# SYNCC-IN/hyperscanning-signal-analysis

Measured on AMD Instinct MI355X. Metric: MVAR+ffDTF windows/sec, 2x32-ch dyad p=8, 256 freqs, higher is better.
Workload: dtype f64; 1 GPU; C2: 1 dyad(s)/GPU, 2x32 ch @500 Hz, 10 min, 2 s windows 50% overlap (599 windows per dyad), MVAR p=8, 256 freqs 0.5-128 Hz; dyads_per_gpu=1, k1=hop blocks summed once, shared by the overlapping windows (hop 500), k2=block Levinson-Whittle recursion, one workgroup per window, one launch, normalisation=inside K3 (rows of window w by workgroups of window w+lag), parallelism=dyad-sharded x1, gather=none

## Files before the change

hyperscanning_signal_analysis_amd/csrc/tf_inv.hip:

```cpp
#include "hmv_common.h"
#include "hmv_kernels.h"

namespace hmv {

#ifndef HMV_K3_WGS
#define HMV_K3_WGS 4
#endif

#ifndef HMV_ROW_LOADS_SC1
#define HMV_ROW_LOADS_SC1 0
#endif

#define HMV_LDS_FENCE()                                     \
  do {                                                      \
    __builtin_amdgcn_fence(__ATOMIC_RELEASE, "wavefront");  \
    __builtin_amdgcn_wave_barrier();                        \
    __builtin_amdgcn_fence(__ATOMIC_ACQUIRE, "wavefront");  \
  } while (0)

#ifdef HMV_STAMP
#define HMV_T(idx)                                                                     \
  do {                                                                                 \
    __builtin_amdgcn_sched_barrier(0);                                                 \
    unsigned long long t_;                                                             \
    asm volatile("s_memtime %0\n\ts_waitcnt lgkmcnt(0)" : "=s"(t_)::"memory");          \
    __builtin_amdgcn_sched_barrier(0);                                                 \
    tsum[idx] += t_ - tlast;                                                           \
    tlast = t_;                                                                        \
  } while (0)
#else
#define HMV_T(idx) do { } while (0)
#endif

template <int NT>
struct TfLds {
  static constexpr int MP = 16 * NT;
  static constexpr int NRING = 3;
  static constexpr int PBUF = MP * 5;
  static constexpr int NBUF = MP * 4;
  static constexpr int SROW = 8;
  static constexpr int SWAPB = NT * 32;
  static constexpr int RSUM = NT * MP / 2;
  static constexpr int TOTAL = PBUF + NRING * NBUF + SROW + SWAPB + RSUM;
};

typedef double f64x2 __attribute__((ext_vector_type(2)));
__device__ __forceinline__ void store_sc1_b128(double* p, f64x2 v) {
  asm volatile("global_store_dwordx4 %0, %1, off sc1\n\ts_nop 1" ::"v"(p), "v"(v) : "memory");
}
__device__ __forceinline__ void store_sc1_b64(double* p, double v) {
  asm volatile("global_store_dwordx2 %0, %1, off sc1" ::"v"(p), "v"(v) : "memory");
}

template <int NT>
struct NormLds {
  static constexpr int MP = 16 * NT;
  static constexpr int FC = 16, JC = (MP % 32 == 0) ? 32 : 16, TS = JC + 1;
  static constexpr int DOUBLES = NT * FC * TS + 5 * MP;
};

template <int NT>
__device__ __forceinline__ void window_denominators(const TfArgs& a, int item, double* lds, const int tid) {
  constexpr int MP = 16 * NT;
  using N = NormLds<NT>;
  double* dpart = lds + NT * N::FC * N::TS;
  const int F = a.F, t = tid;
  const int ty = t / MP, tx = t - ty * MP;
  const double* rs = a.rowsum + (size_t)item * F * MP + tx;
  const int fq = (F + 3) >> 2;
  const int f1 = min(F, (ty + 1) * fq);
  double acc = 0.0;
  int f = ty * fq;
  for (; f + 16 <= f1; f += 16) {
    double v[16];
#pragma unroll
    for (int k = 0; k < 16; ++k) v[k] = rs[(size_t)(f + k) * MP];
#pragma unroll
    for (int k = 0; k < 16; ++k) acc += v[k];
  }
  for (; f < f1; ++f) acc += rs[(size_t)f * MP];
  dpart[ty * MP + tx] = acc;
  __syncthreads();
  if (t < MP) {
    const double d = ((dpart[t] + dpart[MP + t]) + dpart[2 * MP + t]) + dpart[3 * MP + t];
    store_sc1_b64(a.den + (size_t)item * MP + t, d);
  }
}

template <int NT>
__device__ __forceinline__ void normalise_row(const TfArgs& a, int item, int i, double* lds, const int tid) {
  constexpr int MP = 16 * NT;
  using N = NormLds<NT>;
  constexpr int FC = N::FC, JC = N::JC, TS = N::TS;
  constexpr int J2 = JC / 2, FR = 64 / J2, NL = FC / FR, NQ = JC / 8, NJC = MP / JC, D = 4;
  const int F = a.F, m = a.m;
  const int l = tid & 63, wv = uni(tid >> 6);
  double* tile = lds + wv * (FC * TS);
  const double r = 1.0 / __hip_atomic_load(a.den + (size_t)item * MP + i, __ATOMIC_RELAXED, __HIP_MEMORY_SCOPE_AGENT);
  const int total = (F / FC) * NJC;
  const int fr = l / J2, j2 = l - fr * J2;
  const int f2 = l & 7, jr = l >> 3;
#if !HMV_ROW_LOADS_SC1
  const double* Pw = a.P + ((size_t)item * MP + i) * F * MP + (size_t)fr * MP + 2 * j2;
#endif
  double* ow = a.ff + ((size_t)item * m + i) * m * F + (size_t)jr * F + 2 * f2;
#if HMV_ROW_LOADS_SC1
  const double* slab = a.P + ((size_t)item * MP + i) * F * MP;
  const __amdgpu_buffer_rsrc_t rs = __builtin_amdgcn_make_buffer_rsrc(const_cast<double*>(slab), 0, F * MP * 8, 0x00020000);
  const int off0 = (fr * MP + 2 * j2) * 8;
#endif
  auto issue = [&](f64x2 (&v)[NL], int u) __attribute__((always_inline)) {
    if (u < total) {
      const int jc = u % NJC, f0 = (u / NJC) * FC;
#if HMV_ROW_LOADS_SC1
      const int off = off0 + (f0 * MP + jc * JC) * 8;
#pragma unroll
      for (int k = 0; k < NL; ++k)
        v[k] = __builtin_bit_cast(f64x2, __builtin_amdgcn_raw_buffer_load_b128(rs, off + k * FR * MP * 8, 0, 16 ));
#else
      const double* src = Pw + (size_t)f0 * MP + jc * JC;
#pragma unroll
      for (int k = 0; k < NL; ++k)
        v[k] = __builtin_nontemporal_load(reinterpret_cast<const f64x2*>(src + (size_t)(k * FR) * MP));
#endif
    }
  };
  auto drain = [&](const f64x2 (&v)[NL], int u) __attribute__((always_inline)) {
    if (u < total) {
      const int jc = u % NJC, f0 = (u / NJC) * FC, j0 = jc * JC;
#pragma unroll
      for (int k = 0; k < NL; ++k) {
        double* w = tile + (fr + k * FR) * TS + 2 * j2;
        w[0] = v[k].x;
        w[1] = v[k].y;
      }
      HMV_LDS_FENCE();
      double* dst = ow + (size_t)j0 * F + f0;
#pragma unroll
      for (int q = 0; q < NQ; ++q) {
        const double x0 = tile[(2 * f2) * TS + jr + 8 * q], x1 = tile[(2 * f2 + 1) * TS + jr + 8 * q];
        f64x2 o;
        o.x = x0 * r;
        o.y = x1 * r;
        if (j0 + jr + 8 * q < m) __builtin_nontemporal_store(o, reinterpret_cast<f64x2*>(dst + (size_t)(8 * q) * F));
      }
      HMV_LDS_FENCE();
    }
  };
  f64x2 buf[D][NL];
  static_for<D>([&](auto dc) __attribute__((always_inline)) { issue(buf[decltype(dc)::value], wv + NT * decltype(dc)::value); });
  for (int u = wv; u < total; u += NT * D) {
    static_for<D>([&](auto dc) __attribute__((always_inline)) {
      constexpr int d = decltype(dc)::value;
      drain(buf[d], u + NT * d);
      issue(buf[d], u + NT * (d + D));
    });
  }
}

template <int NT>
__device__ __forceinline__ void band_row(const TfArgs& a, int item, int i, double* lds, const int lds_doubles, const int tid) {
  constexpr int MP = 16 * NT, NBP = 5, D = 4;
  const int F = a.F, m = a.m, nb = a.nb;
  const int l = tid & 63, wv = uni(tid >> 6);
  const int c = l & 15, jl = 8 * wv + 2 * (l >> 4);
  const double r = 1.0 / __hip_atomic_load(a.den + (size_t)item * MP + i, __ATOMIC_RELAXED, __HIP_MEMORY_SCOPE_AGENT);
  const int fit = lds_doubles / F;
  const int nbp = fit < NBP ? fit : NBP;
  const int nk = F >> 5;
  for (int b0 = 0; b0 < nb; b0 += nbp) {
    __syncthreads();
    for (int e = tid; e < nbp * F; e += 64 * NT) {
      const int b = e / F, f = e - b * F, bb = b0 + b;
      lds[e] = (bb < nb && f >= a.band_lo[bb] && f < a.band_hi[bb]) ? 1.0 : 0.0;
    }
    __syncthreads();
    const double* wl = lds + 2 * c;
// ... 68 lines not shown
    else normalise_row<NT>(a, item, i, lds, (int)threadIdx.x);
    __syncthreads();
  }
}

template <int NT, bool GEN, bool BANDS = true>
__device__ __forceinline__ void tf_outputs(const TfArgs& a, const int item, const int f, const long long gw, const int w,
                                           const int wv, double (&re)[NT][4], double (&im)[NT][4], double2* smem,
                                           double* rsum, const int* s_orig, int* s_flag, const double* s_det
#ifdef HMV_STAMP
                                           , unsigned long long (&tsum)[8], unsigned long long& tlast
#endif
) {
  constexpr int MP = 16 * NT, NG = NT;
  using L = TfLds<NT>;
  constexpr int NR = L::NRING;
  int& s_info = *s_flag;
  int lo;
  asm volatile("v_mbcnt_lo_u32_b32 %0, -1, 0\n\tv_mbcnt_hi_u32_b32 %0, -1, %0" : "=v"(lo));
  const int rowo = 4 * ((lo >> 2) & 3) + (lo >> 4), jo = lo & 3;
  const int tid = 64 * wv + lo;
  int oc[4];
#pragma unroll
  for (int Jl = 0; Jl < 4; ++Jl) oc[Jl] = s_orig[4 * (Jl * NT + w) + jo];
  if (w == 0 && lo == 0) {
    a.info[gw] = s_info;
    if constexpr (GEN) {
      if (a.detph) {
        a.detph[2 * gw] = s_det[0];
        a.detph[2 * gw + 1] = s_det[1];
      }
    }
  }

  if (a.H) {
    double2* Ho = reinterpret_cast<double2*>(a.H) + (size_t)gw * MP * MP + (size_t)rowo * MP;
#pragma unroll
    for (int Ig = 0; Ig < NG; ++Ig)
#pragma unroll
      for (int Jl = 0; Jl < 4; ++Jl) Ho[(size_t)(16 * Ig) * MP + oc[Jl]] = make_double2(re[Ig][Jl], im[Ig][Jl]);
  }
  if (a.P) {
    double* rs = rsum + w * MP + rowo;
    const bool publish = !GEN && (a.ff != nullptr || a.bands != nullptr) && item < a.fuse_items;
    if (!publish) {
      double* Po = a.P + (size_t)gw * MP * MP + (size_t)rowo * MP;
#pragma unroll
      for (int Ig = 0; Ig < NG; ++Ig) {
        double acc = 0.0;
#pragma unroll
        for (int Jl = 0; Jl < 4; ++Jl) {
          const double v = re[Ig][Jl] * re[Ig][Jl] + im[Ig][Jl] * im[Ig][Jl];
          Po[(size_t)(16 * Ig) * MP + oc[Jl]] = v;
          acc += v;
        }
        acc += dpp_f64<0xB1>(acc);
        acc += dpp_f64<0x4E>(acc);
        if (jo == 0) rs[16 * Ig] = acc;
      }
      __syncthreads();
      if (w == 0 && lo < MP) {
        double t = 0.0;
#pragma unroll
        for (int ww = 0; ww < NT; ++ww) t += rsum[ww * MP + lo];
        a.rowsum[(size_t)gw * MP + lo] = t;
      }
    } else {
      constexpr int G = (NT == 3) ? 1 : (NT == 4 ? 2 : NT), TS = MP + 2, C2 = MP / 2, CNT = 16 * G * C2;
      static_assert(16 * G * TS <= 2 * (L::PBUF + NR * L::NBUF + L::SROW + L::SWAPB), "publish tile overlaps the row sums");
      double* tile = reinterpret_cast<double*>(smem);
      double* Pg = a.P + (size_t)item * MP * a.F * MP + (size_t)f * MP;
      static_for<NG / G>([&](auto pc) __attribute__((always_inline)) {
        constexpr int pass = decltype(pc)::value;
        if (pass > 0) __syncthreads();
        static_for<G>([&](auto gc) __attribute__((always_inline)) {
          constexpr int g = decltype(gc)::value, Ig = pass * G + g;
          double acc = 0.0;
#pragma unroll
          for (int Jl = 0; Jl < 4; ++Jl) {
            const double v = re[Ig][Jl] * re[Ig][Jl] + im[Ig][Jl] * im[Ig][Jl];
            tile[(16 * g + rowo) * TS + oc[Jl]] = v;
            acc += v;
          }
          acc += dpp_f64<0xB1>(acc);
          acc += dpp_f64<0x4E>(acc);
          if (jo == 0) rs[16 * Ig] = acc;
        });
        __syncthreads();
#pragma unroll
        for (int idx = tid; idx < CNT; idx += 64 * NT) {
          const int row = idx / C2, c2 = idx - row * C2;
          const f64x2 v = *reinterpret_cast<const f64x2*>(tile + row * TS + 2 * c2);
          store_sc1_b128(Pg + (size_t)(16 * G * pass + row) * a.F * MP + 2 * c2, v);
        }
      });
      if (w == 0 && lo < MP) {
        double t = 0.0;
#pragma unroll
        for (int ww = 0; ww < NT; ++ww) t += rsum[ww * MP + lo];
        store_sc1_b64(a.rowsum + (size_t)gw * MP + lo, t);
      }
    }
  }
  HMV_T(4);

  if constexpr (!GEN) {
    if (a.ff != nullptr || a.bands != nullptr) {
      static_assert(NormLds<NT>::DOUBLES <= 2 * L::TOTAL, "normaliser tiles do not fit the inversion's LDS block");
      double* nlds = reinterpret_cast<double*>(smem);
      if (item < a.fuse_items) {
        asm volatile("s_waitcnt vmcnt(0)" ::: "memory");
        __syncthreads();
        if (tid == 0) {
          const int old = __hip_atomic_fetch_add(a.wcount + item, 1, __ATOMIC_RELAXED, __HIP_MEMORY_SCOPE_AGENT);
          const int last = (old == a.F - 1) ? 1 : 0;
          if (last) {
            __builtin_amdgcn_fence(__ATOMIC_ACQUIRE, "agent");
            asm volatile("s_waitcnt vmcnt(0)" ::: "memory");
          }
          s_info = last;
        }
        __syncthreads();
        HMV_T(5);
        if (s_info != 0) {
          window_denominators<NT>(a, item, nlds, tid);
          asm volatile("s_waitcnt vmcnt(0)" ::: "memory");
          __syncthreads();
          if (tid == 0) __hip_atomic_store(a.ready + item, 1, __ATOMIC_RELAXED, __HIP_MEMORY_SCOPE_AGENT);
        }
      }
      const int wl = item - a.lag;
      if (wl >= 0 && wl < a.fuse_items - a.lag && f < a.m) {
        __syncthreads();
        if (tid == 0) {
          const int rdy = __hip_atomic_load(a.ready + wl, __ATOMIC_RELAXED, __HIP_MEMORY_SCOPE_AGENT);
          if (!rdy) {
            for (int i = f; i < a.m; i += a.F) {
              const int pos = __hip_atomic_fetch_add(a.missed, 1, __ATOMIC_RELAXED, __HIP_MEMORY_SCOPE_AGENT);
              a.missed[1 + pos] = wl * MP + i;
            }
          }
          s_info = rdy;
        }
        __syncthreads();
        HMV_T(6);
        if (s_info != 0) {
          if (BANDS && a.bands) {
            if constexpr (BANDS)
              for (int i = f; i < a.m; i += a.F) band_row<NT>(a, wl, i, nlds, 2 * L::TOTAL, tid);
          } else {
            for (int i = f; i < a.m; i += a.F) normalise_row<NT>(a, wl, i, nlds, tid);
          }
        }
      }
    }
  }
#ifdef HMV_STAMP
  HMV_T(7);
  if (a.stamps && lo == 0) {
    for (int k = 0; k < 8; ++k) a.stamps[(gw * NT + wv) * 8 + k] = tsum[k];
  }
#endif
}

template <int NT, bool GEN>
__global__ void __launch_bounds__(64 * NT, (NT == 4) ? HMV_K3_WGS : 2) tf_inv_kernel(TfArgs a) {
  constexpr int MP = 16 * NT, NG = NT, NSTEP = MP / 4;
  using L = TfLds<NT>;
  constexpr int NR = L::NRING;
  __shared__ double2 smem[L::TOTAL];
  __shared__ int s_orig[MP];
  __shared__ __attribute__((aligned(16))) int s_swp[NR][4];
  __shared__ int s_info;
  __shared__ double s_det[2];

  const int l = lane_id();
  const int wv = uni(threadIdx.x >> 6);
  const unsigned bid = blockIdx.x + (unsigned)a.item0 * (unsigned)a.F;
  const int w = (wv + (int)((bid * 2654435761u) >> 20)) % NT;
  const int item = uni((int)(bid / (unsigned)a.F));
  const int f = uni((int)(bid - (unsigned)item * (unsigned)a.F));
  const long long gw = (long long)item * a.F + f;
  const int p = a.p;
  const int i = l >> 4, b = (l >> 2) & 3, j = l & 3;
  const int rowl = 4 * b + i;
  const int colw = 4 * w + j;

  double2* Pbuf = smem;
  double2* Nbuf = Pbuf + L::PBUF;
  double2* Srow = Nbuf + NR * L::NBUF;
  double2* swapb = Srow + L::SROW + wv * 32;
// ... 611 lines not shown
```

hyperscanning_signal_analysis_amd/_lib.py:

```python
from __future__ import annotations

import ctypes
import os
from ctypes import POINTER, c_char_p, c_double, c_int, c_int32, c_int64, c_void_p

_HERE = os.path.dirname(os.path.abspath(__file__))
LIB_PATH = os.path.join(_HERE, "libhypermvar.so")

SIGNATURES = {
    "hmv_version": (c_int, []),
    "hmv_last_error": (c_char_p, []),
    "hmv_pad": (c_int, [c_int]),
    "hmv_set_tuning": (c_int, [c_int, c_int64]),
    "hmv_get_tuning": (c_int64, [c_int]),
    "hmv_yw_workspace_doubles": (c_int64, [c_int, c_int]),
    "hmv_lagcov_f64": (c_int, [c_void_p, c_int64, c_int64, c_void_p, c_void_p, c_int64, c_int, c_int, c_int,
                               c_void_p, c_void_p]),
    "hmv_lagcov_regular_workspace_doubles": (c_int64, [c_int64, c_int, c_int, c_int64, c_int]),
    "hmv_lagcov_regular_f64": (c_int, [c_void_p, c_int64, c_int64, c_int64, c_int64, c_int64, c_int, c_int, c_int,
                                       c_void_p, c_void_p, c_void_p]),
    "hmv_yw_solve_f64": (c_int, [c_void_p, c_int64, c_int, c_int, c_void_p, c_void_p, c_void_p, c_void_p,
                                 c_void_p, c_int64, c_void_p]),
    "hmv_yw_routes_i32": (c_int, [c_void_p, c_int64, c_int, c_int, c_void_p, c_void_p]),
    "hmv_twiddles_f64": (c_int, [c_void_p, c_int, c_double, c_int, c_void_p, c_void_p]),
# ... 107 lines not shown
    "hmv_surrogate_phase_c128": (c_int, [c_void_p, c_int64, c_void_p, c_int, c_int, c_int, c_void_p, c_void_p]),
    "hmv_null_accumulate_f64": (c_int, [c_void_p, c_void_p, c_void_p, c_void_p, c_int64, c_int, c_int, c_int] + [c_void_p] * 12),
    "hmv_residuals_workspace_bytes": (c_int64, [c_int64, c_int, c_int]),
    "hmv_residuals_f64": (c_int, [c_void_p, c_int64, c_int64, c_void_p, c_void_p, c_int64, c_int, c_int, c_int, c_void_p,
                                  c_void_p, c_int64, c_void_p, c_int64, c_void_p]),
    "hmv_whiteness_f64": (c_int, [c_void_p, c_int64, c_int, c_int, c_int, c_double] + [c_void_p] * 6),
    "hmv_model_validation_workspace_bytes": (c_int64, [c_int64, c_int, c_int, c_int, c_int]),
    "hmv_model_validation_f64": (c_int, [c_void_p, c_int64, c_int64, c_void_p, c_void_p, c_int64, c_int, c_int, c_int,
                                         c_void_p, c_int, c_double] + [c_void_p] * 7 + [c_int64, c_void_p, c_int64, c_int64,
                                                                                       c_void_p]),
    "hmv_decimate_out_len": (c_int64, [c_int64, c_int]),
    "hmv_decimate_tile": (c_int, [c_int, c_int]),
    "hmv_decimate_fir_f64": (c_int, [c_void_p, c_int64, c_int64, c_int64, c_int64, c_int, c_int, c_void_p, c_int, c_void_p,
                                     c_int64, c_int64, c_void_p]),
    "hmv_phase_sync_c128": (c_int, [c_void_p, c_int64, c_int64, c_int64, c_int64, c_int, c_void_p, c_void_p, c_int64, c_int, c_int,
                                    c_void_p, c_void_p, c_void_p, c_void_p, c_void_p]),
}

FLAG_UNFUSED_NORM = 1
FLAG_YW_TILED = 2
FLAG_YW_ONE_LAUNCH = 4
FLAG_DIRECT_LAGCOV = 8
FLAG_YW_PIVOTED = 16
MEASURE_FFDTF = 0
MEASURE_DDTF = 1
MEASURE_GPDC = 2
CRITERIA = {"AIC": 0, "HQ": 1, "SC": 2}
TUNE_NORM_LAG = 1
TUNE_LAG_GROUP = 2
TUNE_K3_FORM = 3
TUNE_YW_FORM = 4
TUNE_K3_LDS_PAD = 5
TUNE_K3_SPLIT = 6
MAX_DECIMATE = 32
MAX_DECIMATE_TAPS = 641
PHASE_UNIT = 0
PHASE_RAW = 1


_lib = None


class HypermvarLibraryError(ImportError):
    pass


def load():
    global _lib
    if _lib is not None:
        return _lib
    global LIB_PATH
    LIB_PATH = os.environ.get("HYPERMVAR_LIB", LIB_PATH)
    if not os.path.exists(LIB_PATH):
        raise HypermvarLibraryError(
            f"{LIB_PATH} not found: build the HIP library first "
            f"(python -c 'import __graft_entry__ as g; g.build()' or make -C {_HERE}/csrc). "
            "There is no CPU fallback for the MVAR/ffDTF path.")
    lib = ctypes.CDLL(LIB_PATH)
    for name, (res, args) in SIGNATURES.items():
        try:
            fn = getattr(lib, name)
        except AttributeError as e:
            raise HypermvarLibraryError(f"{LIB_PATH} does not export {name}") from e
        fn.restype = res
        fn.argtypes = args
    _lib = lib
# ... 11 lines not shown
```

hyperscanning_signal_analysis_amd/csrc/capi.hip:

```cpp
#include "../../include/hypermvar.h"
#include "hmv_kernels.h"

#include <atomic>
#include <cmath>
#include <cstdio>
#include <cstdlib>
#include <cstring>

namespace {
thread_local char g_err[256] = "";

int fail(int code, const char* msg) {
  snprintf(g_err, sizeof(g_err), "%s", msg);
  return code;
}
int refuse(const char* who, int code, const char* msg) {
  snprintf(g_err, sizeof(g_err), "%s: %s", who, msg);
  return code;
}
int pad_of(int m) { return (m < 1 || m > HMV_MAX_CHANNELS) ? -1 : ((m + 15) / 16) * 16; }
inline hipStream_t S(void* s) { return reinterpret_cast<hipStream_t>(s); }
inline size_t align256(size_t b) { return (b + 255) & ~size_t(255); }

constexpr int N_TUNE = 7;
// ... 619 lines not shown
  return w;
}
struct BgcWs {
  size_t off_B, off_C, off_D, off_cst, off_Ra, off_Rb, off_arr, off_Vra, off_Vrb, off_ir, off_full, total;
};
BgcWs bgc_layout(size_t front, int64_t chunk, int m, int p, int F, int split, bool bands, bool time, bool spectral = true) {
  BgcWs w;
  size_t o = front;
  const hmv::BgcPads pd = hmv::bgc_pads(m, split);
  const size_t mp = (size_t)pad_of(m), mpa = (size_t)pd.mpa, mpb = (size_t)pd.mpb, nsp = (size_t)pd.nsp, pp = (size_t)p + 1;
  w.off_B = o;      if (spectral) o += align256(sizeof(double) * chunk * pp * mp * mp);
  w.off_C = o;      if (spectral) o += align256(sizeof(double) * chunk * 2 * pp * nsp * nsp);
  w.off_D = o;      if (spectral) o += align256(sizeof(double) * chunk * 2 * pp * nsp * nsp);
  w.off_cst = o;    if (spectral) o += align256(sizeof(double) * chunk * 2);
  w.off_Ra = o;     if (time) o += align256(sizeof(double) * chunk * pp * mpa * mpa);
  w.off_Rb = o;     if (time) o += align256(sizeof(double) * chunk * pp * mpb * mpb);
  w.off_arr = o;    if (time) o += align256(sizeof(double) * chunk * nsp * nsp * p);
  w.off_Vra = o;    if (time) o += align256(sizeof(double) * chunk * mpa * mpa);
  w.off_Vrb = o;    if (time) o += align256(sizeof(double) * chunk * mpb * mpb);
  w.off_ir = o;     if (time) o += align256(sizeof(int32_t) * chunk * 2);
  w.off_full = o;   if (bands) o += align256(sizeof(double) * chunk * 2 * F);
  w.total = o;
  return w;
}
int64_t sliding_bytes(int64_t chunk, int m, int p, int F, int n_bands = 0, bool spectra = false, int measure = MEAS_FFDTF,
                      int64_t q_tiles = -1) {
  const int mp = pad_of(m);
  if (mp < 0 || chunk < 1 || p < 1 || p > HMV_MAX_ORDER || F < 1 || n_bands < 0 || measure < MEAS_FFDTF ||
      measure > MEAS_GPDC)
    return -1;
  return (int64_t)sliding_layout(chunk, mp, p, F, n_bands > 0, spectra, measure, q_tiles).total;
}
struct ForkJoin {
  hipEvent_t fork = nullptr, join = nullptr;
};
ForkJoin* fork_join_events() {
  constexpr int MAXDEV = 64;
  thread_local ForkJoin tl[MAXDEV];
  int dev = 0;
  if (hipGetDevice(&dev) != hipSuccess || dev < 0 || dev >= MAXDEV) return nullptr;
  ForkJoin& e = tl[dev];
  if (!e.fork) {
    if (hipEventCreateWithFlags(&e.fork, hipEventDisableTiming) != hipSuccess) return nullptr;
    if (hipEventCreateWithFlags(&e.join, hipEventDisableTiming) != hipSuccess) return nullptr;
  }
  return &e;
}
int64_t k3_split_point(int64_t c, int mp, int64_t lag) {
  const int64_t t = hmv::tuning(HMV_TUNE_K3_SPLIT);
  int64_t c0 = t;
  if (t < 0) return 0;
  if (t == 0) {
    constexpr int MAXDEV = 64;
    struct Shape { int cus = 0, occ[4] = {0, 0, 0, 0}; };
    thread_local Shape tl[MAXDEV];
    int dev = 0;
    if (hipGetDevice(&dev) != hipSuccess || dev < 0 || dev >= MAXDEV || mp < 16 || mp > 64) return 0;
    Shape& d = tl[dev];
    int& occ = d.occ[mp / 16 - 1];
    if (d.cus == 0 && hipDeviceGetAttribute(&d.cus, hipDeviceAttributeMultiprocessorCount, dev) != hipSuccess) d.cus = -1;
    if (occ == 0 && (occ = hmv::yw_lwr_occupancy(mp)) == 0) occ = -1;
    if (d.cus < 1 || occ < 1) {
      (void)hipGetLastError();
      return 0;
    }
    const int64_t k = c / d.cus, r = c % d.cus;
    if (k < 1 || k >= occ || r == 0) return 0;
    c0 = c - r;
  }
  return (c0 >= lag && c0 < c) ? c0 : 0;
}
}

int64_t hmv_sliding_workspace_bytes(int64_t chunk, int m, int p, int F) { return sliding_bytes(chunk, m, p, F); }

namespace {
struct MixDesc {
  const double* Rt;
  const double* W;
  const double* scale;
  int64_t n_trials, n_win, n_mix;
};
struct BgcDesc {
  int split;
  double* time;
  int32_t* info_red;
  int32_t* info_gc;
  int want = 3;
  double* red_out = nullptr;
  const double* red_base = nullptr;
  const int32_t* info_red_base = nullptr;
};
struct Items {
  const double* x;
  int64_t rec_stride, ld;
  const int64_t* item_rec;
  const int64_t* item_start;
  int64_t n_items;
  int m, n, p;
};
struct Grid { int64_t hop, first, nwin, T; };
struct Spectral { const double* freqs; int F; double fs; };
struct Output {
// ... 39 lines not shown
  Run run;
  OrderSel sel = {};
  const EnsDesc* ens = nullptr;
  const PairDesc* pairs = nullptr;
  const MixDesc* mix = nullptr;
  const BgcDesc* bgc = nullptr;
};

int measure_request(const char* who, int measure, int n_bands, const double* S_out, FitOut& fit, int crit = 0) {
  if (measure < HMV_MEASURE_FFDTF || measure > HMV_MEASURE_GPDC)
    return refuse(who, -4, "measure must be HMV_MEASURE_FFDTF, _DDTF or _GPDC");
  if (crit < 0 || crit > 2) return refuse(who, -5, "criterion must be 0 (AIC), 1 (HQ) or 2 (SC)");
  if (n_bands < 0) return refuse(who, -4, "n_bands must be >= 0");
  if (S_out && (measure != HMV_MEASURE_FFDTF || n_bands != 0))
    return refuse(who, -4, "spectra come with the full ffDTF only");
  if (measure == HMV_MEASURE_GPDC) { fit.info_tf = nullptr; fit.pivot_tau = 1.0; }
  return 0;
}
int need_output(const char* who, const void* out, int64_t n_items) {
  return (!out && n_items != 0) ? refuse(who, -4, "null pointer / empty grid") : 0;
}
int need_output_after_sizes(const char* who, const Items& it, const void* out) {
  const bool sizes_ok = pad_of(it.m) >= 0 && it.p >= 1 && it.p <= HMV_MAX_ORDER && it.n > it.p;
  return sizes_ok ? need_output(who, out, it.n_items) : 0;
}
int64_t measure_bytes(int measure, int64_t chunk, int m, int p, int F, int n_bands, int64_t q_tiles) {
  const bool spectra = (n_bands == -1 && measure == HMV_MEASURE_FFDTF);
  return sliding_bytes(chunk, m, p, F, spectra ? 0 : n_bands, spectra, measure, q_tiles);
}

struct TwoStreams {
  hipStream_t st0 = nullptr, st1 = nullptr;
  ForkJoin* ev = nullptr;
  int fork() const {
    const int hrc = (int)hipEventRecord(ev->fork, st0);
    return hrc ? hrc : (int)hipStreamWaitEvent(st1, ev->fork, 0);
  }
  int record_join() const {
    const int hrc = (int)hipEventRecord(ev->join, st1);
    if (hrc) (void)hipStreamSynchronize(st1);
    return hrc;
  }
  int wait_join(hipEvent_t join) const {
    const int hrc = (int)hipStreamWaitEvent(st0, join, 0);
    if (hrc) (void)hipStreamSynchronize(st1);
    return hrc;
  }
  int join() const {
    const int hrc = record_join();
    return hrc ? hrc : wait_join(ev->join);
  }
  void finish(hmv::TfSplit& sp) const {
    if (sp.join && !sp.joined) (void)wait_join(sp.join);
    sp.joined = true;
  }
};

struct SlidingPlan {
  bool empty = false;
  int mp = 0;
  size_t t = 0, ws_item = 0;
  bool automatic = false, bands = false, k3_bands = false, bgc_spec = false, bgc_time = false;
  bool regular = false, ens_shared = false;
  bool ldl = false, from_tiles = false;
  bool half_split = false, k3_split = false;
  TwoStreams fj;
  SlidingWs w{};
  BgcWs gw{};
  char* base = nullptr;
  double *R = nullptr, *Qb = nullptr, *ws = nullptr, *ar = nullptr, *V = nullptr, *den = nullptr, *tw = nullptr;
// ... 96 lines not shown

int sliding_k1(const SlidingArgs& a, const SlidingPlan& pl, const Chunk& ch) {
  const Items& it = a.it;
  const int64_t i0 = ch.i0, c = ch.c;
  hipStream_t st = pl.fj.st0;
  const K1In in{it.x, it.rec_stride, it.ld, it.item_rec, it.item_start, it.m, it.n, it.p};
  if (a.ens) {
    const hmv::LagcovEnsArgs ea = ens_args(in, *a.ens, i0, c, pl.R, pl.ens_shared ? pl.Qb : nullptr, a.grid.hop, a.grid.nwin);
    return a.ens->split ? hmv::launch_lagcov_ensemble_split(ea, pl.mp, st)
                        : hmv::launch_lagcov_ensemble(ea, pl.mp, pl.ens_shared, st);
  }
  if (a.pairs) return hmv::launch_lagcov_pairs(pairs_args(in, *a.pairs, i0, c, pl.R), pl.mp, st);
  if (a.mix) {
    hmv::LagcovMixArgs ma{};
    ma.Rt = a.mix->Rt; ma.W = a.mix->W; ma.scale = a.mix->scale; ma.n_trials = a.mix->n_trials; ma.n_win = a.mix->n_win;
    ma.it0 = i0; ma.n_items = c; ma.m = it.m; ma.m_pad = pl.mp; ma.p = it.p; ma.R = pl.R;
    return hmv::launch_lagcov_mix(ma, st);
  }
  if (!pl.regular)
    return hmv_lagcov_f64(it.x, it.rec_stride, it.ld, it.item_rec + i0, it.item_start + i0, c, it.m, it.n, it.p, pl.R, st);
  const Grid& g = a.grid;
  const size_t stack = (size_t)(it.p + 1) * pl.t;
  int rc = 0;
  for (int64_t k = i0; k < i0 + c && rc == 0;) {
    const int64_t rec = k / g.nwin, w0 = k - rec * g.nwin;
    const int64_t run = ((g.nwin - w0) < (i0 + c - k)) ? (g.nwin - w0) : (i0 + c - k);
    rc = hmv_lagcov_regular_f64(it.x + rec * it.rec_stride, it.ld, g.T, g.first + w0 * g.hop, g.hop, run, it.m, it.n, it.p,
                                pl.R + (size_t)(k - i0) * stack, pl.Qb, st);
    k += run;
  }
  return rc;
}

int sliding_k2(const SlidingArgs& a, const SlidingPlan& pl, const Chunk& ch, hmv::TfSplit& sp) {
  const Items& it = a.it;
  const int64_t flags = a.run.flags, c = ch.c;
  const int mp = pl.mp;
  const TwoStreams& fj = pl.fj;
  auto part = [&](int64_t k0, int64_t cnt, int64_t yw_flags) {
    return yw_args(pl.R + (size_t)k0 * (it.p + 1) * pl.t, cnt, it.m, it.p, pl.ws + (size_t)k0 * pl.ws_item,
                   ch.ar + (size_t)k0 * pl.t * it.p, ch.V + (size_t)k0 * pl.t, a.fit.info_yw + ch.i0 + k0, yw_flags);
  };
  sp = hmv::TfSplit{};
  if (pl.automatic)
    return hmv::launch_yw_auto(part(0, c, flags),
                               yw_auto_args(it.n, a.sel.crit, a.sel.order_out + ch.i0,
                                            a.sel.crit_out ? a.sel.crit_out + (size_t)ch.i0 * it.p : nullptr), mp, fj.st0);
  if (!pl.from_tiles) {
    const int64_t yw_flags = pl.yw_flags(flags, mp, c);
    const int64_t c0 = (pl.half_split && (yw_flags & HMV_FLAG_YW_TILED) && c >= 16) ? (c + 1) / 2 : c;
    if (c0 < c) {
      if (const int hrc = fj.fork()) return hrc;
      int rc = hmv::launch_yw(part(c0, c - c0, yw_flags), mp, fj.st1);
      const int hrc = fj.join();
      if (!rc) rc = hrc;
      if (rc) return rc;
    }
    return hmv::launch_yw(part(0, c0, yw_flags), mp, fj.st0);
  }
  const int64_t s0 = pl.k3_split ? k3_split_point(c, mp, norm_lag_items(mp, a.spec.F)) : 0;
  hmv::YwArgs ya = part(0, s0 ? s0 : c, flags);
  ya.no_emit = 1;
  int rc = hmv::launch_yw(ya, mp, fj.st0);
  if (rc || !s0) return rc;
  if (const int hrc = fj.fork()) return hrc;
  hmv::YwArgs yb = part(s0, c - s0, flags);
  yb.no_emit = 1;
  rc = hmv::launch_yw(yb, mp, fj.st1);
  if (const int hrc = fj.record_join()) return rc ? rc : hrc;
  sp.c0 = s0;
  sp.join = fj.ev->join;
  return rc;
}

int sliding_bgc(const SlidingArgs& a, const SlidingPlan& pl, const Chunk& ch) {
  const Items& it = a.it;
  const BgcDesc& g = *a.bgc;
  const BgcWs& gw = pl.gw;
  const int64_t i0 = ch.i0, c = ch.c, flags = a.run.flags;
  hipStream_t st0 = pl.fj.st0;
  const int na = g.split, nb2 = it.m - na, F = a.spec.F;
  int rc = 0;
  hmv::BgcArgs ga{};
  ga.want = g.want;
  if (pl.bgc_time) {
    ga.red.time = g.time + (size_t)i0 * 4; ga.red.info_red = g.info_red + (size_t)i0 * 2;
    ga.red.red_out = g.red_out ? g.red_out + (size_t)i0 * 2 : nullptr;
  }
  if (pl.bgc_time && g.red_base) {
    ga.red.red_base = g.red_base; ga.red.info_red_base = g.info_red_base;
    ga.red.base_a = ll(a.pairs->base_a + i0); ga.red.base_b = ll(a.pairs->base_b + i0);
  } else if (pl.bgc_time) {
    double* Ra = pl.at(gw.off_Ra);
// ... 46 lines not shown
                       o.n_bands, pl.den, Hc, a.fit.info_tf + (size_t)i0 * F, a.fit.pivot_tau, pl.tfws, pl.tfws_bytes,
                       a.run.flags,
                       ch.last ? a.run.ev_k3_start : nullptr, ch.last ? a.run.ev_k3_stop : nullptr, st0,
                       pl.from_tiles ? pl.ws : nullptr, &sp);
  if (!rc && a.measure == MEAS_DDTF) {
    hmv::DdtfArgs da{};
    da.ar = ch.ar; da.V = ch.V; da.info_yw = a.fit.info_yw + i0;
    da.B = pl.at(pl.w.off_B); da.G = pl.at(pl.w.off_G);
    da.freqs = a.spec.freqs; da.fs = a.spec.fs; da.ff = full_c; da.out = full_c;
    da.n_items = c; da.F = F; da.m = m; da.p = it.p;
    rc = hmv::launch_ddtf_sliding(da, pl.mp, st0);
  }
  if (!rc && pl.bands && !pl.k3_bands)
    rc = hmv::launch_band_sums(full_c, lo, hi, out_c, c * (long long)m * m, F, o.n_bands, st0);
  if (!rc && o.S_out) {
    hmv::SpecArgs sa;
    sa.H = Hc; sa.V = ch.V; sa.S = nullptr; sa.S_mmf = o.S_out + (size_t)i0 * m * m * F * 2;
    sa.n_items = c; sa.F = F; sa.m = m; sa.sym = 1;
    rc = hmv::launch_spectra(sa, pl.mp, st0);
  }
  return rc;
}

int sliding_impl(const SlidingArgs& a) {
  SlidingPlan pl;
  int rc = sliding_plan(a, pl);
  if (rc || pl.empty) return rc;
  if (pl.bgc_spec) rc = hmv_twiddles_f64(a.spec.freqs, a.spec.F, a.spec.fs, a.it.p, pl.tw, a.run.stream);
  const int64_t n = a.it.n_items, chunk = a.run.chunk;
  hmv::TfSplit sp{};
  for (int64_t i0 = 0; i0 < n && rc == 0; i0 += chunk) {
    const Chunk ch{i0, n - i0 < chunk ? n - i0 : chunk, a.fit.ar_out ? a.fit.ar_out + (size_t)i0 * pl.t * a.it.p : pl.ar,
                   a.fit.V_out ? a.fit.V_out + (size_t)i0 * pl.t : pl.V, i0 + chunk >= n};
    rc = sliding_k1(a, pl, ch);
    if (!rc) rc = sliding_k2(a, pl, ch, sp);
    if (!rc) rc = a.measure == MEAS_BGC ? sliding_bgc(a, pl, ch) : sliding_measure(a, pl, ch, sp);
    pl.fj.finish(sp);
  }
  return rc;
}
}

int64_t hmv_sliding_bands_workspace_bytes(int64_t chunk, int m, int p, int F) { return sliding_bytes(chunk, m, p, F, 1); }

int hmv_sliding_ffdtf_f64(const double* x, int64_t rec_stride, int64_t ld, const int64_t* item_rec,
                          const int64_t* item_start, int64_t n_items, int m, int n, int p,
                          const double* freqs, int F, double fs, double* ffdtf, double* ar_out, double* V_out,
                          int32_t* info_yw, int32_t* info_tf, void* workspace, int64_t workspace_bytes,
                          int64_t chunk, double pivot_tau, int64_t flags, int64_t grid_hop, int64_t grid_first,
                          int64_t grid_nwin, int64_t grid_T, void* ev_k3_start, void* ev_k3_stop, void* stream,
                          void* aux_stream) {
  return sliding_impl({"hmv_sliding_ffdtf_f64", MEAS_FFDTF, {x, rec_stride, ld, item_rec, item_start, n_items, m, n, p},
                       {grid_hop, grid_first, grid_nwin, grid_T}, {freqs, F, fs}, output(ffdtf),
                       {ar_out, V_out, info_yw, info_tf, pivot_tau},
                       {workspace, workspace_bytes, chunk, flags, stream, aux_stream, ev_k3_start, ev_k3_stop}});
}

int hmv_sliding_ffdtf_bands_f64(const double* x, int64_t rec_stride, int64_t ld, const int64_t* item_rec,
                                const int64_t* item_start, int64_t n_items, int m, int n, int p,
                                const double* freqs, int F, double fs, double* band_out, const int32_t* bin_lo,
                                const int32_t* bin_hi, int n_bands, double* ar_out, double* V_out,
                                int32_t* info_yw, int32_t* info_tf, void* workspace, int64_t workspace_bytes,
                                int64_t chunk, double pivot_tau, int64_t flags, int64_t grid_hop, int64_t grid_first,
                                int64_t grid_nwin, int64_t grid_T, void* ev_k3_start, void* ev_k3_stop, void* stream,
                                void* aux_stream) {
  const char* who = "hmv_sliding_ffdtf_bands_f64";
  if (int rc = need_output(who, band_out, n_items)) return rc;
  return sliding_impl({who, MEAS_FFDTF, {x, rec_stride, ld, item_rec, item_start, n_items, m, n, p},
// ... 585 lines not shown
```

include/hypermvar.h:

```cpp
#ifndef HYPERMVAR_H
#define HYPERMVAR_H

#include <stdint.h>

#ifdef __cplusplus
extern "C" {
#endif

#define HMV_VERSION 160
#define HMV_MAX_CHANNELS 64
#define HMV_MAX_ORDER 32

int hmv_version(void);
const char* hmv_last_error(void);
int hmv_pad(int m);
#define HMV_TUNE_NORM_LAG 1
#define HMV_TUNE_LAG_GROUP 2
#define HMV_TUNE_K3_FORM 3
#define HMV_TUNE_YW_FORM 4
#define HMV_TUNE_K3_LDS_PAD 5
#define HMV_TUNE_K3_SPLIT 6
int hmv_set_tuning(int key, int64_t value);
int64_t hmv_get_tuning(int key);
int64_t hmv_yw_workspace_doubles(int m, int p);

int hmv_lagcov_f64(const double* x, int64_t rec_stride, int64_t ld,
                   const int64_t* item_rec, const int64_t* item_start, int64_t n_items,
                   int m, int n, int p, double* R, void* stream);

#define HMV_MAX_HOPS_PER_WINDOW 8
int64_t hmv_lagcov_regular_workspace_doubles(int64_t n_win, int m, int n, int64_t hop, int p);
int hmv_lagcov_regular_f64(const double* x, int64_t ld, int64_t T, int64_t first, int64_t hop, int64_t n_win,
                           int m, int n, int p, double* R, double* workspace, void* stream);

int hmv_yw_routes_i32(const double* ws, int64_t n_items, int m, int p, int32_t* route, void* stream);
int hmv_yw_solve_f64(const double* R, int64_t n_items, int m, int p, double* ws,
                     double* ar, double* V, double* vq_logdet, int32_t* info, int64_t flags, void* stream);

int hmv_twiddles_f64(const double* freqs, int F, double fs, int p, double* tw, void* stream);

int64_t hmv_tf_workspace_doubles(int64_t n_items, int m, int p);
int hmv_tf_f64(const double* ar, int64_t n_items, int m, int p, const double* tw, int F,
               double* P, double* rowsum, double* H, double* A, int32_t* info,
               double pivot_tau, double* ws, void* stream);

int hmv_ffdtf_norm_f64(const double* P, const double* rowsum, double* den, double* out,
                       int64_t n_items, int F, int m, int normalise, void* stream);

int hmv_transpose_c128(const double* in, double* out, int64_t n_items, int F, int m, void* stream);

int hmv_spectra_f64(const double* H, const double* V, double* S, int64_t n_items, int m, int F, void* stream);
int hmv_spectra_mmf_f64(const double* H, const double* V, double* S, int64_t n_items, int m, int F, void* stream);

int hmv_pack_c128(const double* in, double* out, int64_t n_items, int F, int m, void* stream);
// ... 249 lines not shown
```

Measured before the change: 59380 windows/s.

## Normalise lagged window before arrival counting and drop barriers in publish path

Moves the lagged-window normalisation ahead of the per-window arrival counter. The ready flag is read early and the missed list is filled during the publish pass, so normalisation overlaps the outstanding P stores instead of waiting behind a block-wide barrier. Arrival is now counted per wave through an LDS atomic on s_info, which replaces a __syncthreads, and each wave reads out its own publish rows so no barrier is needed before reusing LDS. Address arithmetic is also rewritten to use scalar-base plus 32-bit vector-offset global stores and loads with explicit LDS address spaces. The cost is more intricate synchronisation: LDS reuse rests on the new row-ownership static assertions, and s_info now carries both the ready bit and the wave count.

```diff
diff --git a/hyperscanning_signal_analysis_amd/csrc/tf_inv.hip b/hyperscanning_signal_analysis_amd/csrc/tf_inv.hip
--- a/hyperscanning_signal_analysis_amd/csrc/tf_inv.hip
+++ b/hyperscanning_signal_analysis_amd/csrc/tf_inv.hip
@@ -45,8 +45,23 @@
 };
 
 typedef double f64x2 __attribute__((ext_vector_type(2)));
-__device__ __forceinline__ void store_sc1_b128(double* p, f64x2 v) {
-  asm volatile("global_store_dwordx4 %0, %1, off sc1\n\ts_nop 1" ::"v"(p), "v"(v) : "memory");
+typedef double __attribute__((address_space(3))) lds_f64;
+typedef f64x2 __attribute__((address_space(3))) lds_f64x2;
+typedef const char __attribute__((address_space(1)))* gcbytes;
+typedef char __attribute__((address_space(1)))* gbytes;
+__device__ __forceinline__ gcbytes sbase_of(unsigned long long base, size_t ubytes) {
+  unsigned long long sb = base + ubytes;
+  asm volatile("" : "+s"(sb));
+  return reinterpret_cast<gcbytes>(sb);
+}
+__device__ __forceinline__ gcbytes sbase_of(const double* base, size_t ubytes) {
+  return sbase_of(reinterpret_cast<unsigned long long>(base), ubytes);
+}
+__device__ __forceinline__ gcbytes sbase_of(gcbytes base, size_t ubytes) {
+  return sbase_of(reinterpret_cast<unsigned long long>(base), ubytes);
+}
+__device__ __forceinline__ void store_sc1_b128(gcbytes sbase, unsigned voff, f64x2 v) {
+  asm volatile("global_store_dwordx4 %0, %1, %2 sc1\n\ts_nop 1" ::"v"(voff), "v"(v), "s"(sbase) : "memory");
 }
 __device__ __forceinline__ void store_sc1_b64(double* p, double v) {
   asm volatile("global_store_dwordx2 %0, %1, off sc1" ::"v"(p), "v"(v) : "memory");
@@ -101,9 +116,13 @@
   const int fr = l / J2, j2 = l - fr * J2;
   const int f2 = l & 7, jr = l >> 3;
 #if !HMV_ROW_LOADS_SC1
-  const double* Pw = a.P + ((size_t)item * MP + i) * F * MP + (size_t)fr * MP + 2 * j2;
-#endif
-  double* ow = a.ff + ((size_t)item * m + i) * m * F + (size_t)jr * F + 2 * f2;
+  const double* Ps = a.P + ((size_t)item * MP + i) * F * MP;
+  const unsigned lin = (unsigned)(fr * MP + 2 * j2) * 8u;
+#endif
+  const double* os = a.ff + ((size_t)item * m + i) * m * F;
+  const unsigned lout = (unsigned)(jr * F + 2 * f2) * 8u;
+  lds_f64* tw = (lds_f64*)tile + (fr * TS + 2 * j2);
+  const lds_f64* tr = (lds_f64*)tile + (2 * f2 * TS + jr);
 #if HMV_ROW_LOADS_SC1
   const double* slab = a.P + ((size_t)item * MP + i) * F * MP;
   const __amdgpu_buffer_rsrc_t rs = __builtin_amdgcn_make_buffer_rsrc(const_cast<double*>(slab), 0, F * MP * 8, 0x00020000);
@@ -118,10 +137,11 @@
       for (int k = 0; k < NL; ++k)
         v[k] = __builtin_bit_cast(f64x2, __builtin_amdgcn_raw_buffer_load_b128(rs, off + k * FR * MP * 8, 0, 16 ));
 #else
-      const double* src = Pw + (size_t)f0 * MP + jc * JC;
+      const gcbytes src = sbase_of(Ps, (size_t)(unsigned)(f0 * MP + jc * JC) * 8u);
 #pragma unroll
       for (int k = 0; k < NL; ++k)
-        v[k] = __builtin_nontemporal_load(reinterpret_cast<const f64x2*>(src + (size_t)(k * FR) * MP));
+        v[k] = __builtin_nontemporal_load(
+            reinterpret_cast<const f64x2 __attribute__((address_space(1)))*>(src + k * FR * MP * 8 + (size_t)lin));
 #endif
     }
   };
@@ -130,19 +150,19 @@
       const int jc = u % NJC, f0 = (u / NJC) * FC, j0 = jc * JC;
 #pragma unroll
       for (int k = 0; k < NL; ++k) {
-        double* w = tile + (fr + k * FR) * TS + 2 * j2;
-        w[0] = v[k].x;
-        w[1] = v[k].y;
+        tw[k * FR * TS] = v[k].x;
+        tw[k * FR * TS + 1] = v[k].y;
       }
       HMV_LDS_FENCE();
-      double* dst = ow + (size_t)j0 * F + f0;
 #pragma unroll
       for (int q = 0; q < NQ; ++q) {
-        const double x0 = tile[(2 * f2) * TS + jr + 8 * q], x1 = tile[(2 * f2 + 1) * TS + jr + 8 * q];
+        const double x0 = tr[8 * q], x1 = tr[TS + 8 * q];
         f64x2 o;
         o.x = x0 * r;
         o.y = x1 * r;
-        if (j0 + jr + 8 * q < m) __builtin_nontemporal_store(o, reinterpret_cast<f64x2*>(dst + (size_t)(8 * q) * F));
+        const gbytes dst = const_cast<gbytes>(sbase_of(os, ((size_t)(unsigned)(j0 + 8 * q) * (unsigned)F + (unsigned)f0) * 8u));
+        if (j0 + jr + 8 * q < m)
+          __builtin_nontemporal_store(o, reinterpret_cast<f64x2 __attribute__((address_space(1)))*>(dst + (size_t)lout));
       }
       HMV_LDS_FENCE();
     }
@@ -277,6 +297,20 @@
       }
     }
   }
+  constexpr int PG = (NT == 3) ? 1 : (NT == 4 ? 2 : NT), PTS = MP + 2, PC2 = MP / 2, PCNT = 16 * PG * PC2;
+  constexpr int PNIT = PCNT / (64 * NT);
+  constexpr bool PWROWS = (64 % PC2 == 0) && ((16 * PG) % NT == 0);
+  constexpr int PRI = PWROWS ? 64 / PC2 : 1, PRW = 16 * PG / NT;
+  constexpr bool OWN_ROWS = PWROWS && NT > 1 && PRW * PTS == NormLds<NT>::FC * NormLds<NT>::TS;
+  static_assert(PCNT % (64 * NT) == 0 && (!PWROWS || PNIT * PRI == PRW), "publish read-out does not tile the pass");
+  static_assert(NT != 4 || OWN_ROWS, "the 64-channel row tiles no longer coincide with the waves' read-out rows");
+  [[maybe_unused]] int wl = 0, rdy_early = 0;
+  [[maybe_unused]] bool carries = false;
+  if constexpr (!GEN) {
+    wl = item - a.lag;
+    carries = (a.ff != nullptr || a.bands != nullptr) && wl >= 0 && wl < a.fuse_items - a.lag && f < a.m;
+    if (carries && tid == 0) rdy_early = __hip_atomic_load(a.ready + wl, __ATOMIC_RELAXED, __HIP_MEMORY_SCOPE_AGENT);
+  }
 
   if (a.H) {
     double2* Ho = reinterpret_cast<double2*>(a.H) + (size_t)gw * MP * MP + (size_t)rowo * MP;
@@ -311,10 +345,14 @@
         a.rowsum[(size_t)gw * MP + lo] = t;
       }
     } else {
-      constexpr int G = (NT == 3) ? 1 : (NT == 4 ? 2 : NT), TS = MP + 2, C2 = MP / 2, CNT = 16 * G * C2;
+      constexpr int G = PG, TS = PTS, C2 = PC2;
       static_assert(16 * G * TS <= 2 * (L::PBUF + NR * L::NBUF + L::SROW + L::SWAPB), "publish tile overlaps the row sums");
-      double* tile = reinterpret_cast<double*>(smem);
-      double* Pg = a.P + (size_t)item * MP * a.F * MP + (size_t)f * MP;
+      lds_f64* tile = (lds_f64*)reinterpret_cast<double*>(smem);
+      const double* Pg = a.P + (size_t)item * MP * a.F * MP + (size_t)f * MP;
+      const unsigned rbytes = (unsigned)a.F * (unsigned)(MP * 8);
+      lds_f64* wp[4];
+#pragma unroll
+      for (int Jl = 0; Jl < 4; ++Jl) wp[Jl] = tile + (rowo * TS + oc[Jl]);
       static_for<NG / G>([&](auto pc) __attribute__((always_inline)) {
         constexpr int pass = decltype(pc)::value;
         if (pass > 0) __syncthreads();
@@ -324,7 +362,7 @@
 #pragma unroll
           for (int Jl = 0; Jl < 4; ++Jl) {
             const double v = re[Ig][Jl] * re[Ig][Jl] + im[Ig][Jl] * im[Ig][Jl];
-            tile[(16 * g + rowo) * TS + oc[Jl]] = v;
+            wp[Jl][16 * g * TS] = v;
             acc += v;
           }
           acc += dpp_f64<0xB1>(acc);
@@ -332,11 +370,42 @@
           if (jo == 0) rs[16 * Ig] = acc;
         });
         __syncthreads();
-#pragma unroll
-        for (int idx = tid; idx < CNT; idx += 64 * NT) {
-          const int row = idx / C2, c2 = idx - row * C2;
-          const f64x2 v = *reinterpret_cast<const f64x2*>(tile + row * TS + 2 * c2);
-          store_sc1_b128(Pg + (size_t)(16 * G * pass + row) * a.F * MP + 2 * c2, v);
+        if constexpr (pass == 0) {
+          if (tid == 0) {
+            if (carries && !rdy_early) {
+              for (int i = f; i < a.m; i += a.F) {
+                const int pos = __hip_atomic_fetch_add(a.missed, 1, __ATOMIC_RELAXED, __HIP_MEMORY_SCOPE_AGENT);
+                a.missed[1 + pos] = wl * MP + i;
+              }
+            }
+            s_info = rdy_early;
+          }
+        }
+        if constexpr (PWROWS) {
+          const unsigned lr = (unsigned)lo / C2, c2 = (unsigned)lo % C2;
+          const lds_f64* rp = tile + ((PRW * wv + lr) * TS + 2 * c2);
+          const unsigned voff = lr * rbytes + c2 * 16u;
+          gcbytes sb = sbase_of(Pg, (size_t)(unsigned)(16 * G * pass + PRW * wv) * rbytes);
+          f64x2 v[PNIT];
+#pragma unroll
+          for (int it = 0; it < PNIT; ++it) v[it] = *reinterpret_cast<const lds_f64x2*>(rp + it * PRI * TS);
+#pragma unroll
+          for (int it = 0; it < PNIT; ++it) {
+            store_sc1_b128(sb, voff, v[it]);
+            if (it + 1 < PNIT) sb = sbase_of(sb, (size_t)(PRI * rbytes));
+          }
+        } else {
+          const gcbytes sb = sbase_of(Pg, (size_t)(unsigned)(16 * G * pass) * rbytes);
+          f64x2 v[PNIT];
+          unsigned voff[PNIT];
+#pragma unroll
+          for (int it = 0; it < PNIT; ++it) {
+            const unsigned idx = (unsigned)tid + 64 * NT * it, row = idx / C2, c2 = idx - row * C2;
+            v[it] = *reinterpret_cast<const lds_f64x2*>(tile + (row * TS + 2 * c2));
+            voff[it] = row * rbytes + c2 * 16u;
+          }
+#pragma unroll
+          for (int it = 0; it < PNIT; ++it) store_sc1_b128(sb, voff[it], v[it]);
         }
       });
       if (w == 0 && lo < MP) {
@@ -351,19 +420,32 @@
 
   if constexpr (!GEN) {
     if (a.ff != nullptr || a.bands != nullptr) {
-      static_assert(NormLds<NT>::DOUBLES <= 2 * L::TOTAL, "normaliser tiles do not fit the inversion's LDS block");
+      static_assert(NormLds<NT>::DOUBLES <= 2 * (L::TOTAL - L::RSUM), "normaliser tiles reach the row sums, which wave w = 0 may still be reading");
       double* nlds = reinterpret_cast<double*>(smem);
       if (item < a.fuse_items) {
+        if constexpr (!OWN_ROWS) __syncthreads();
+        HMV_T(6);
+        if (carries && (uni(s_info) & 1) != 0) {
+          if (BANDS && a.bands) {
+            if constexpr (BANDS)
+              for (int i = f; i < a.m; i += a.F) band_row<NT>(a, wl, i, nlds, 2 * L::TOTAL, tid);
+          } else {
+            for (int i = f; i < a.m; i += a.F) normalise_row<NT>(a, wl, i, nlds, tid);
+          }
+        }
+        HMV_T(7);
         asm volatile("s_waitcnt vmcnt(0)" ::: "memory");
-        __syncthreads();
-        if (tid == 0) {
-          const int old = __hip_atomic_fetch_add(a.wcount + item, 1, __ATOMIC_RELAXED, __HIP_MEMORY_SCOPE_AGENT);
-          const int last = (old == a.F - 1) ? 1 : 0;
-          if (last) {
-            __builtin_amdgcn_fence(__ATOMIC_ACQUIRE, "agent");
-            asm volatile("s_waitcnt vmcnt(0)" ::: "memory");
+        if (lo == 0) {
+          const int before = __hip_atomic_fetch_add(&s_info, 2, __ATOMIC_RELAXED, __HIP_MEMORY_SCOPE_WORKGROUP) >> 1;
+          if (before == NT - 1) {
+            const int old = __hip_atomic_fetch_add(a.wcount + item, 1, __ATOMIC_RELAXED, __HIP_MEMORY_SCOPE_AGENT);
+            const int last = (old == a.F - 1) ? 1 : 0;
+            if (last) {
+              __builtin_amdgcn_fence(__ATOMIC_ACQUIRE, "agent");
+              asm volatile("s_waitcnt vmcnt(0)" ::: "memory");
+            }
+            s_info = last;
           }
-          s_info = last;
         }
         __syncthreads();
         HMV_T(5);
@@ -374,34 +456,9 @@
           if (tid == 0) __hip_atomic_store(a.ready + item, 1, __ATOMIC_RELAXED, __HIP_MEMORY_SCOPE_AGENT);
         }
       }
-      const int wl = item - a.lag;
-      if (wl >= 0 && wl < a.fuse_items - a.lag && f < a.m) {
-        __syncthreads();
-        if (tid == 0) {
-          const int rdy = __hip_atomic_load(a.ready + wl, __ATOMIC_RELAXED, __HIP_MEMORY_SCOPE_AGENT);
-          if (!rdy) {
-            for (int i = f; i < a.m; i += a.F) {
-              const int pos = __hip_atomic_fetch_add(a.missed, 1, __ATOMIC_RELAXED, __HIP_MEMORY_SCOPE_AGENT);
-              a.missed[1 + pos] = wl * MP + i;
-            }
-          }
-          s_info = rdy;
-        }
-        __syncthreads();
-        HMV_T(6);
-        if (s_info != 0) {
-          if (BANDS && a.bands) {
-            if constexpr (BANDS)
-              for (int i = f; i < a.m; i += a.F) band_row<NT>(a, wl, i, nlds, 2 * L::TOTAL, tid);
-          } else {
-            for (int i = f; i < a.m; i += a.F) normalise_row<NT>(a, wl, i, nlds, tid);
-          }
-        }
-      }
     }
   }
 #ifdef HMV_STAMP
-  HMV_T(7);
   if (a.stamps && lo == 0) {
     for (int k = 0; k < 8; ++k) a.stamps[(gw * NT + wv) * 8 + k] = tsum[k];
   }
```

Measured after the change: 59920 windows/s (median of 6 runs). About the same (+0.9%).

## Split sliding chunk at CU count and overlap tail K1/K2 on aux stream

Applied to the files above, without the earlier changes.

Adds a 'front' split mode: when the chunk has more windows than CUs, the first CU-count windows and the tail are processed on two streams. Hop-block sums for the head run first, then the tail's sums, combine and Yule-Walker solve run on the second stream while the head's combine and solve run on the main stream, joined before K3 finishes. The intent is to fill the partial wave of workgroups and overlap K1 with K2 across streams instead of running them serially. It adds extra events and launches and a tuning bit to disable it, and it risks contention between the two streams.

```diff
diff --git a/hyperscanning_signal_analysis_amd/_lib.py b/hyperscanning_signal_analysis_amd/_lib.py
--- a/hyperscanning_signal_analysis_amd/_lib.py
+++ b/hyperscanning_signal_analysis_amd/_lib.py
@@ -163,6 +163,7 @@
 TUNE_YW_FORM = 4
 TUNE_K3_LDS_PAD = 5
 TUNE_K3_SPLIT = 6
+K3_SPLIT_NO_FRONT = 1 << 19
 MAX_DECIMATE = 32
 MAX_DECIMATE_TAPS = 641
 PHASE_UNIT = 0
diff --git a/hyperscanning_signal_analysis_amd/csrc/capi.hip b/hyperscanning_signal_analysis_amd/csrc/capi.hip
--- a/hyperscanning_signal_analysis_amd/csrc/capi.hip
+++ b/hyperscanning_signal_analysis_amd/csrc/capi.hip
@@ -675,7 +675,7 @@
   return (int64_t)sliding_layout(chunk, mp, p, F, n_bands > 0, spectra, measure, q_tiles).total;
 }
 struct ForkJoin {
-  hipEvent_t fork = nullptr, join = nullptr;
+  hipEvent_t fork = nullptr, join = nullptr, front = nullptr;
 };
 ForkJoin* fork_join_events() {
   constexpr int MAXDEV = 64;
@@ -686,32 +686,43 @@
   if (!e.fork) {
     if (hipEventCreateWithFlags(&e.fork, hipEventDisableTiming) != hipSuccess) return nullptr;
     if (hipEventCreateWithFlags(&e.join, hipEventDisableTiming) != hipSuccess) return nullptr;
+    if (hipEventCreateWithFlags(&e.front, hipEventDisableTiming) != hipSuccess) return nullptr;
   }
   return &e;
 }
-int64_t k3_split_point(int64_t c, int mp, int64_t lag) {
-  const int64_t t = hmv::tuning(HMV_TUNE_K3_SPLIT);
+struct SplitPoint {
+  int64_t c0;
+  bool front;
+};
+SplitPoint k3_split_point(int64_t c, int mp, int64_t lag, bool can_front) {
+  int64_t t = hmv::tuning(HMV_TUNE_K3_SPLIT);
+  if (t < 0) return {};
+  if (t >= HMV_K3_SPLIT_NO_FRONT) {
+    t -= HMV_K3_SPLIT_NO_FRONT;
+    can_front = false;
+  }
   int64_t c0 = t;
-  if (t < 0) return 0;
   if (t == 0) {
     constexpr int MAXDEV = 64;
     struct Shape { int cus = 0, occ[4] = {0, 0, 0, 0}; };
     thread_local Shape tl[MAXDEV];
     int dev = 0;
-    if (hipGetDevice(&dev) != hipSuccess || dev < 0 || dev >= MAXDEV || mp < 16 || mp > 64) return 0;
+    if (hipGetDevice(&dev) != hipSuccess || dev < 0 || dev >= MAXDEV || mp < 16 || mp > 64) return {};
     Shape& d = tl[dev];
     int& occ = d.occ[mp / 16 - 1];
     if (d.cus == 0 && hipDeviceGetAttribute(&d.cus, hipDeviceAttributeMultiprocessorCount, dev) != hipSuccess) d.cus = -1;
     if (occ == 0 && (occ = hmv::yw_lwr_occupancy(mp)) == 0) occ = -1;
     if (d.cus < 1 || occ < 1) {
       (void)hipGetLastError();
-      return 0;
+      return {};
     }
     const int64_t k = c / d.cus, r = c % d.cus;
-    if (k < 1 || k >= occ || r == 0) return 0;
+    if (can_front && c > d.cus && k < occ && d.cus >= lag) return {d.cus, true};
+    if (k < 1 || k >= occ || r == 0) return {};
     c0 = c - r;
-  }
-  return (c0 >= lag && c0 < c) ? c0 : 0;
+    can_front = false;
+  }
+  return (c0 >= lag && c0 < c) ? SplitPoint{c0, can_front} : SplitPoint{};
 }
 }
 
@@ -817,10 +828,12 @@
 struct TwoStreams {
   hipStream_t st0 = nullptr, st1 = nullptr;
   ForkJoin* ev = nullptr;
-  int fork() const {
-    const int hrc = (int)hipEventRecord(ev->fork, st0);
-    return hrc ? hrc : (int)hipStreamWaitEvent(st1, ev->fork, 0);
-  }
+  int fork(hipEvent_t at) const {
+    const int hrc = (int)hipEventRecord(at, st0);
+    return hrc ? hrc : (int)hipStreamWaitEvent(st1, at, 0);
+  }
+  int fork() const { return fork(ev->fork); }
+  int fork_front() const { return fork(ev->front); }
   int record_join() const {
     const int hrc = (int)hipEventRecord(ev->join, st1);
     if (hrc) (void)hipStreamSynchronize(st1);
@@ -983,15 +996,75 @@
   return rc;
 }
 
-int sliding_k2(const SlidingArgs& a, const SlidingPlan& pl, const Chunk& ch, hmv::TfSplit& sp) {
+hmv::YwArgs k2_part(const SlidingArgs& a, const SlidingPlan& pl, const Chunk& ch, int64_t k0, int64_t cnt, int64_t yw_flags) {
+  const Items& it = a.it;
+  return yw_args(pl.R + (size_t)k0 * (it.p + 1) * pl.t, cnt, it.m, it.p, pl.ws + (size_t)k0 * pl.ws_item,
+                 ch.ar + (size_t)k0 * pl.t * it.p, ch.V + (size_t)k0 * pl.t, a.fit.info_yw + ch.i0 + k0, yw_flags);
+}
+
+bool front_cut_ok(const SlidingArgs& a, const SlidingPlan& pl, const Chunk& ch) {
+  if (a.ens || a.pairs || a.mix) return false;
+  return !pl.regular || ch.i0 % a.grid.nwin + ch.c <= a.grid.nwin;
+}
+SplitPoint sliding_split(const SlidingArgs& a, const SlidingPlan& pl, const Chunk& ch) {
+  if (!pl.k3_split || !pl.from_tiles) return {};
+  return k3_split_point(ch.c, pl.mp, norm_lag_items(pl.mp, a.spec.F), front_cut_ok(a, pl, ch));
+}
+
+int sliding_front(const SlidingArgs& a, const SlidingPlan& pl, const Chunk& ch, int64_t c0, hmv::TfSplit& sp) {
+  const Items& it = a.it;
+  const Grid& g = a.grid;
+  const TwoStreams& fj = pl.fj;
+  const int64_t i0 = ch.i0, c = ch.c;
+  const size_t stack = (size_t)(it.p + 1) * pl.t;
+  const int k = pl.regular ? (int)(it.n / g.hop) : 1;
+  const int64_t rec = pl.regular ? i0 / g.nwin : 0;
+  const double* x = it.x + rec * it.rec_stride;
+  const int64_t first = pl.regular ? g.first + (i0 - rec * g.nwin) * g.hop : 0;
+  auto sums = [&](int64_t k0, int64_t k1, hipStream_t st) {
+    if (!pl.regular)
+      return hmv_lagcov_f64(it.x, it.rec_stride, it.ld, it.item_rec + i0 + k0, it.item_start + i0 + k0, k1 - k0, it.m, it.n,
+                            it.p, pl.R + (size_t)k0 * stack, st);
+    const int64_t b0 = k0 ? k0 + k - 1 : 0;
+    hmv::LagcovArgs la{};
+    la.x = x; la.ld = it.ld; la.n_items = k1 + k - 1 - b0; la.m = it.m; la.n = (int)g.hop; la.p = it.p;
+    la.R = pl.Qb + (size_t)b0 * stack;
+    la.blocks = 1; la.blk_first = first + b0 * g.hop; la.blk_T = g.T;
+    return hmv::launch_lagcov(la, pl.mp, st);
+  };
+  auto comb = [&](int64_t k0, int64_t k1, hipStream_t st) {
+    if (!pl.regular) return 0;
+    hmv::LagcombArgs ca{};
+    ca.Q = pl.Qb + (size_t)k0 * stack; ca.x = x; ca.ld = it.ld; ca.first = first + k0 * g.hop; ca.hop = g.hop; ca.T = g.T;
+    ca.n_win = k1 - k0; ca.k = k; ca.m = it.m; ca.p = it.p; ca.R = pl.R + (size_t)k0 * stack;
+    return hmv::launch_lagcomb(ca, pl.mp, st);
+  };
+  auto solve = [&](int64_t k0, int64_t k1, hipStream_t st) {
+    hmv::YwArgs ya = k2_part(a, pl, ch, k0, k1 - k0, a.run.flags);
+    ya.no_emit = 1;
+    return hmv::launch_yw(ya, pl.mp, st);
+  };
+  sp = hmv::TfSplit{};
+  int rc = sums(0, c0, fj.st0);
+  if (rc) return rc;
+  if (const int hrc = fj.fork_front()) return hrc;
+  rc = sums(c0, c, fj.st1);
+  if (!rc) rc = comb(c0, c, fj.st1);
+  if (!rc) rc = solve(c0, c, fj.st1);
+  if (const int hrc = fj.record_join()) return rc ? rc : hrc;
+  sp.c0 = c0;
+  sp.join = fj.ev->join;
+  if (!rc) rc = comb(0, c0, fj.st0);
+  if (!rc) rc = solve(0, c0, fj.st0);
+  return rc;
+}
+
+int sliding_k2(const SlidingArgs& a, const SlidingPlan& pl, const Chunk& ch, int64_t s0, hmv::TfSplit& sp) {
   const Items& it = a.it;
   const int64_t flags = a.run.flags, c = ch.c;
   const int mp = pl.mp;
   const TwoStreams& fj = pl.fj;
-  auto part = [&](int64_t k0, int64_t cnt, int64_t yw_flags) {
-    return yw_args(pl.R + (size_t)k0 * (it.p + 1) * pl.t, cnt, it.m, it.p, pl.ws + (size_t)k0 * pl.ws_item,
-                   ch.ar + (size_t)k0 * pl.t * it.p, ch.V + (size_t)k0 * pl.t, a.fit.info_yw + ch.i0 + k0, yw_flags);
-  };
+  auto part = [&](int64_t k0, int64_t cnt, int64_t yw_flags) { return k2_part(a, pl, ch, k0, cnt, yw_flags); };
   sp = hmv::TfSplit{};
   if (pl.automatic)
     return hmv::launch_yw_auto(part(0, c, flags),
@@ -1009,7 +1082,6 @@
     }
     return hmv::launch_yw(part(0, c0, yw_flags), mp, fj.st0);
   }
-  const int64_t s0 = pl.k3_split ? k3_split_point(c, mp, norm_lag_items(mp, a.spec.F)) : 0;
   hmv::YwArgs ya = part(0, s0 ? s0 : c, flags);
   ya.no_emit = 1;
   int rc = hmv::launch_yw(ya, mp, fj.st0);
@@ -1122,8 +1194,13 @@
   for (int64_t i0 = 0; i0 < n && rc == 0; i0 += chunk) {
     const Chunk ch{i0, n - i0 < chunk ? n - i0 : chunk, a.fit.ar_out ? a.fit.ar_out + (size_t)i0 * pl.t * a.it.p : pl.ar,
                    a.fit.V_out ? a.fit.V_out + (size_t)i0 * pl.t : pl.V, i0 + chunk >= n};
-    rc = sliding_k1(a, pl, ch);
-    if (!rc) rc = sliding_k2(a, pl, ch, sp);
+    const SplitPoint s = sliding_split(a, pl, ch);
+    if (s.front) {
+      rc = sliding_front(a, pl, ch, s.c0, sp);
+    } else {
+      rc = sliding_k1(a, pl, ch);
+      if (!rc) rc = sliding_k2(a, pl, ch, s.c0, sp);
+    }
     if (!rc) rc = a.measure == MEAS_BGC ? sliding_bgc(a, pl, ch) : sliding_measure(a, pl, ch, sp);
     pl.fj.finish(sp);
   }
diff --git a/include/hypermvar.h b/include/hypermvar.h
--- a/include/hypermvar.h
+++ b/include/hypermvar.h
@@ -20,6 +20,7 @@
 #define HMV_TUNE_YW_FORM 4
 #define HMV_TUNE_K3_LDS_PAD 5
 #define HMV_TUNE_K3_SPLIT 6
+#define HMV_K3_SPLIT_NO_FRONT (1 << 19)
 int hmv_set_tuning(int key, int64_t value);
 int64_t hmv_get_tuning(int key);
 int64_t hmv_yw_workspace_doubles(int m, int p);
```

Result: faster. 63490 windows/s before, 64360 windows/s after (median of 6 runs) (+1.4%).
